# zhizdev/mvdfusion

Hardware: AMD Instinct MI355X
Metric: denoising-steps/sec (higher is better)
Workload: dtype f16x3 (f16 MFMA operands split hi+lo, 3 partial products, fp32 accumulate); 1 GPU; BASELINE.json configs[1]: V=4 views x 256^2 images (32x32 latents), D=1, 50-step DDIM (eta 1), cfg 2.5, SD1.x UNet 320ch + 10 view-aligned transformers + GridAttn, random-init (deterministic fill) weights; views=4, latent=32, depth_samples=1, parallelism=single GPU, CFG pair batched as 2V, hipgraph=True, gemm_tuning=mvdfusion_amd/tuned/gemm_f16.json: 426 problems; 0 problems tuned in this run

## Files before the change

### include/mvd_hip.h

```cpp
#ifndef MVD_HIP_H
#define MVD_HIP_H
#include <stddef.h>
#include <stdint.h>
#ifdef __cplusplus
extern "C" {
#endif

typedef void* mvd_stream_t;

#define MVD_VERSION 100
#define MVD_PREC_X1 1
#define MVD_PREC_X3 3
#define MVD_PREC_X4 4

int mvd_version(void);
const char* mvd_last_error(void);
int mvd_operand_format(void);

size_t mvd_packed_weight_bytes(int N, int K);
int mvd_pack_linear_weight(const float* w, int N, int K, int ldw, int geglu, float scale, void* packed,
                           mvd_stream_t stream);
int mvd_pack_linear_weight_t(const float* wt, int N, int K, int ldw, float scale, void* packed, mvd_stream_t stream);
int mvd_pack_conv3x3_weight(const float* w, int Cout, int Cin, int cin_pad, float scale, void* packed,
                            mvd_stream_t stream);
// ... 119 lines not shown

int mvd_pixel_cross_attn(const float* q, const float* k, const float* v, void* out_sp, int P, int D, int heads,
                         int dhead, mvd_stream_t stream);

int mvd_unet_input(const float* x, const float* input_latents, void* out_sp, int V, int S, int cpad, int cfg,
                   mvd_stream_t stream);
int mvd_unet_input_scenes(const float* x, const float* input_latents, void* out_sp, int nscene, int V, int S, int cpad, int cfg,
                          mvd_stream_t stream);
int mvd_concat_channels(const float* a, int Ca, const float* b, int Cb, float* out, void* out_sp, int rows, long long* gn_stats,
                        int gn_hw, int gn_groups, mvd_stream_t stream);
int mvd_concat_groupnorm_fits(int Ca, int Cb, int hw, int groups);
int mvd_concat_groupnorm(const float* a, int Ca, const float* b, int Cb, float* out, void* raw_sp, void* y_sp, const float* gamma,
                         const float* beta, long long* gn_stats, int B, int hw, int groups, float eps, int silu, mvd_stream_t stream);
int mvd_area_pool(const float* vol, void* out_sp, int B, int S, int D, int C, int factor, int ldp, mvd_stream_t stream);
int mvd_fill_zero(float* p, size_t n, mvd_stream_t stream);

#define MVD_STEP_STRIDE 8
int mvd_timestep_embedding(const float* steps, const int* iter, const float* freqs, float* out, int dim,
                           mvd_stream_t stream);
int mvd_timestep_embedding_scenes(const float* steps, const int* iter, const float* freqs, float* out, int dim, int nscene,
                                  int steps_scene_stride, mvd_stream_t stream);
int mvd_advance_iter(int* iter, mvd_stream_t stream);

#define MVD_CAM_RECORD 20
#define MVD_TOKEN_DIM 723
#define MVD_TOKEN_LD 736
int mvd_zembed(const float* lat, const float* w, const float* b, float* feat, int N, int S, mvd_stream_t stream);
int mvd_gridattn_tokens(const float* x, const float* depth_noise, const float* steps, const int* iter,
                        const float* grid_lin ,
                        const float* feat, const float* in_feat, const float* cams, const float* in_cam,
                        void* tokens_sp, int V, int q0, int Vq, int S, int D, float depth_scale, float depth_shift,
                        mvd_stream_t stream);
int mvd_gridattn_tokens_scenes(const float* x, const float* depth_noise, const float* steps, const int* iter, const float* grid_lin,
                               const float* feat, const float* in_feat, const float* cams, const float* in_cam, void* tokens_sp,
                               int nscene, int V, int q0, int Vq, int S, int D, float depth_scale, float depth_shift,
                               mvd_stream_t stream);
int mvd_gridattn_tokens_scenes_t(const float* x, const float* depth_noise, const float* steps, const int* iter, const float* grid_lin,
                                 const float* feat, const float* in_feat, const float* cams, const float* in_cam, void* tokens_sp,
                                 int nscene, int V, int q0, int Vq, int S, int D, float depth_scale, float depth_shift,
                                 int steps_scene_stride, mvd_stream_t stream);
int mvd_gridattn_fused_slots(void);
size_t mvd_gridattn_fused_stream_bytes(void);
size_t mvd_gridattn_fused_vec_floats(void);
int mvd_gridattn_fused(const float* x, const float* depth_noise, const float* steps, const int* iter, const float* grid_lin,
                       const float* feat, const float* in_feat, const float* cams, const float* in_cam, const void* wstream,
                       const float* vecs, void* pooled_sp, int V, int q0, int Vq, int S, int D, float depth_scale,
// ... 305 lines not shown
```

### mvdfusion_amd/csrc/elementwise.hip

```cpp
#include "common.hpp"
#include "../../include/mvd_hip.h"

namespace {

__device__ __forceinline__ float act_apply(float v, int act) {
  if (act == MVD_ACT_GELU) return gelu_erf(v);
  if (act == MVD_ACT_SILU) return silu_f(v);
  return v;
}

template <int MR>
__global__ __launch_bounds__(256) void gemv_kernel(const float* __restrict__ W, const float* __restrict__ bias,
                                                   const float* __restrict__ x, float* __restrict__ y, int M, int N, int K, int ldx,
                                                   int ldy, int act_in, int act_out) {
  const int lane = threadIdx.x & 63;
  const int n = blockIdx.x * 4 + (threadIdx.x >> 6);
  if (n >= N) return;
  float acc[MR];
#pragma unroll
  for (int m = 0; m < MR; ++m) acc[m] = 0.f;
  const float* wr = W + (size_t)n * K;
  if ((K & 3) == 0) {
    for (int k = lane * 4; k < K; k += 256) {
      const float4 w4 = *(const float4*)(wr + k);
// ... 266 lines not shown
        acc.z += v.z;
        acc.w += v.w;
      }
    store_sp4(out_sp, e / C4, ldp, c * 4, acc.x * inv, acc.y * inv, acc.z * inv, acc.w * inv);
  }
}

__global__ __launch_bounds__(256) void fill_zero_kernel(float* p, size_t n) {
  for (size_t e = (size_t)blockIdx.x * 256 + threadIdx.x; e < n; e += (size_t)gridDim.x * 256) p[e] = 0.f;
}

__global__ void timestep_embedding_kernel(const float* __restrict__ steps, const int* __restrict__ iter,
                                          const float* __restrict__ freqs, float* __restrict__ out, int dim, int steps_scene_stride) {
  const float t = steps[((size_t)iter[0] + (size_t)blockIdx.x * steps_scene_stride) * MVD_STEP_STRIDE + 0];
  out += (size_t)blockIdx.x * dim;
  const int half = dim / 2;
  for (int i = threadIdx.x; i < half; i += blockDim.x) {
    const float a = t * freqs[i];
    out[i] = cosf(a);
    out[half + i] = sinf(a);
  }
}

__global__ void advance_iter_kernel(int* iter) {
  if (threadIdx.x == 0) iter[0] += 1;
}

__global__ __launch_bounds__(256) void cfg_ddim_kernel(const float* __restrict__ eps_nhwc, int ldc, float* __restrict__ x,
                                                       float* __restrict__ x0, float* __restrict__ eps_out,
                                                       const float* __restrict__ noise, const float* __restrict__ steps,
                                                       const int* __restrict__ iter, int V, int S, int cfg, float cfg_scale,
                                                       int do_update, size_t noise_stride) {
  const int it = iter[0];
  const float* st = steps + (size_t)it * MVD_STEP_STRIDE;
  const float a_t = st[3], a_prev = st[4], sigma = st[5], s1m = st[6], has_noise = st[7];
  const int SS = S * S;
  const size_t total = (size_t)V * 5 * SS;
  for (size_t e = (size_t)blockIdx.x * 256 + threadIdx.x; e < total; e += (size_t)gridDim.x * 256) {
    const int pix = (int)(e % SS);
    const int c = (int)((e / SS) % 5);
    const int b = (int)(e / ((size_t)5 * SS));
    float ep = eps_nhwc[((size_t)b * SS + pix) * ldc + c];
    if (cfg) {
      const float eu = eps_nhwc[((size_t)(V + b) * SS + pix) * ldc + c];
      ep = eu + cfg_scale * (ep - eu);
    }
// ... 54 lines not shown
  if (b > (size_t)cap) b = cap;
  if (b < 1) b = 1;
  return (int)b;
}

}

extern "C" int mvd_gemv(const float* W, const float* bias, const float* x, float* y, int M, int N, int K, int ldx, int ldy,
                        int act_in, int act_out, mvd_stream_t stream) {
  MVD_CHECK_ARG(W && x && y && M > 0 && M <= 16 && N > 0 && K > 0, "mvd_gemv: bad arguments (M <= 16)");
  if ((K & 3) == 0) MVD_CHECK_ARG((ldx & 3) == 0, "mvd_gemv: ldx must be a multiple of 4 when K is");
  hipStream_t s = (hipStream_t)stream;
  dim3 grid(cdiv(N, 4)), block(256);
  if (M <= 1)
    hipLaunchKernelGGL(gemv_kernel<1>, grid, block, 0, s, W, bias, x, y, M, N, K, ldx, ldy, act_in, act_out);
  else if (M <= 4)
    hipLaunchKernelGGL(gemv_kernel<4>, grid, block, 0, s, W, bias, x, y, M, N, K, ldx, ldy, act_in, act_out);
  else
    hipLaunchKernelGGL(gemv_kernel<16>, grid, block, 0, s, W, bias, x, y, M, N, K, ldx, ldy, act_in, act_out);
  MVD_CHECK_LAUNCH("mvd_gemv");
  return 0;
}

extern "C" int mvd_unet_input_scenes(const float* x, const float* input_latents, void* out_sp, int nscene, int V, int S, int cpad, int cfg,
                                     mvd_stream_t stream) {
  MVD_CHECK_ARG(x && input_latents && out_sp && cpad % 32 == 0 && V > 0 && S > 0 && cpad >= 10, "mvd_unet_input: bad arguments");
  MVD_CHECK_ARG(nscene >= 1 && (long long)nscene * V <= 0x3fffffff, "mvd_unet_input_scenes: nscene=%d (>= 1)", nscene);
  const int NV = nscene * V;
  const int nb = cfg ? 2 * NV : NV;
  const size_t total = (size_t)nb * S * S * cpad;
  hipLaunchKernelGGL(unet_input_kernel, dim3(grid_for(total)), dim3(256), 0, (hipStream_t)stream, x, input_latents, (u16*)out_sp, NV, V,
                     S, cpad, nb);
  MVD_CHECK_LAUNCH("mvd_unet_input");
  return 0;
}

extern "C" int mvd_unet_input(const float* x, const float* input_latents, void* out_sp, int V, int S, int cpad, int cfg,
                              mvd_stream_t stream) {
  return mvd_unet_input_scenes(x, input_latents, out_sp, 1, V, S, cpad, cfg, stream);
}

extern "C" int mvd_concat_channels(const float* a, int Ca, const float* b, int Cb, float* out, void* out_sp, int rows,
                                   long long* gn_stats, int gn_hw, int gn_groups, mvd_stream_t stream) {
  if (out_sp) MVD_CHECK_ARG((Ca + Cb) % 32 == 0, "mvd_concat_channels: split-planes output needs (Ca+Cb) %% 32 == 0");
  MVD_CHECK_ARG(a && b && out && rows > 0 && Ca > 0 && Cb > 0 && Ca % 4 == 0 && Cb % 4 == 0,
                "mvd_concat_channels: bad arguments (channel counts must be multiples of 4)");
// ... 59 lines not shown
  if (n == 0) return 0;
  hipLaunchKernelGGL(fill_zero_kernel, dim3(grid_for(n)), dim3(256), 0, (hipStream_t)stream, p, n);
  MVD_CHECK_LAUNCH("mvd_fill_zero");
  return 0;
}

extern "C" int mvd_timestep_embedding(const float* steps, const int* iter, const float* freqs, float* out, int dim,
                                      mvd_stream_t stream) {
  MVD_CHECK_ARG(steps && iter && freqs && out && dim > 0 && dim % 2 == 0, "mvd_timestep_embedding: bad arguments");
  hipLaunchKernelGGL(timestep_embedding_kernel, dim3(1), dim3(256), 0, (hipStream_t)stream, steps, iter, freqs, out, dim, 0);
  MVD_CHECK_LAUNCH("mvd_timestep_embedding");
  return 0;
}

extern "C" int mvd_timestep_embedding_scenes(const float* steps, const int* iter, const float* freqs, float* out, int dim, int nscene,
                                             int steps_scene_stride, mvd_stream_t stream) {
  MVD_CHECK_ARG(steps && iter && freqs && out && dim > 0 && dim % 2 == 0, "mvd_timestep_embedding: bad arguments");
  MVD_CHECK_ARG(nscene >= 1 && nscene <= 65535 && steps_scene_stride >= 0 && (nscene > 1 || steps_scene_stride == 0),
                "mvd_timestep_embedding_scenes: nscene=%d (1 ... 65535), steps_scene_stride=%d (>= 0; 0 when nscene = 1)", nscene,
                steps_scene_stride);
  hipLaunchKernelGGL(timestep_embedding_kernel, dim3(nscene), dim3(256), 0, (hipStream_t)stream, steps, iter, freqs, out, dim,
                     steps_scene_stride);
  MVD_CHECK_LAUNCH("mvd_timestep_embedding_scenes");
  return 0;
}

extern "C" int mvd_advance_iter(int* iter, mvd_stream_t stream) {
  MVD_CHECK_ARG(iter != nullptr, "mvd_advance_iter: null pointer");
  hipLaunchKernelGGL(advance_iter_kernel, dim3(1), dim3(64), 0, (hipStream_t)stream, iter);
  MVD_CHECK_LAUNCH("mvd_advance_iter");
  return 0;
}

extern "C" int mvd_cfg_ddim_update(const float* eps_nhwc, int ldc, float* x, float* x0, float* eps_out,
                                   const float* ddim_noise, size_t noise_stride, const float* steps, const int* iter, int V,
                                   int S, int cfg, float cfg_scale, int do_update, mvd_stream_t stream) {
  MVD_CHECK_ARG(eps_nhwc && steps && iter && V > 0 && S > 0 && ldc >= 5, "mvd_cfg_ddim_update: bad arguments");
  if (do_update) MVD_CHECK_ARG(x && x0 && ddim_noise, "mvd_cfg_ddim_update: update needs x, x0, ddim_noise");
  const size_t total = (size_t)V * 5 * S * S;
  hipLaunchKernelGGL(cfg_ddim_kernel, dim3(grid_for(total)), dim3(256), 0, (hipStream_t)stream, eps_nhwc, ldc, x, x0, eps_out,
                     ddim_noise, steps, iter, V, S, cfg, cfg_scale, do_update, noise_stride);
  MVD_CHECK_LAUNCH("mvd_cfg_ddim_update");
  return 0;
}

extern "C" int mvd_pin_views(float* x, float* x0, const float* known, const float* noise, size_t noise_stride, const float* steps,
// ... 26 lines not shown
```

### mvdfusion_amd/hip.py

```python
import ctypes as C
import os

import torch

_HERE = os.path.dirname(os.path.abspath(__file__))
LIB_PATHS = {"f16": os.path.join(_HERE, "csrc", "libmvd_hip.so"), "bf16": os.path.join(_HERE, "csrc", "libmvd_hip_bf16.so")}
if os.environ.get("MVD_HIP_LIB"):
    LIB_PATHS["f16"] = os.environ["MVD_HIP_LIB"]
LIB_PATH = LIB_PATHS["f16"]
OPERAND_FORMAT = os.environ.get("MVD_OPERAND_FORMAT", "f16")

PREC_X1, PREC_X3, PREC_X4 = 1, 3, 4
PREC_KINDS = ("conv", "skip", "proj", "qkv", "attn", "out", "geglu", "ffproj", "xattn", "ga")


def parse_precision(name):
    base, _, over = name.partition(":")
    names = {"f16": ("f16", PREC_X1), "bf16": ("bf16", PREC_X1), "f16x3": ("f16", PREC_X3), "f16x4": ("f16", PREC_X4),
             "bf16x3": ("bf16", PREC_X3), "bf16x4": ("bf16", PREC_X4)}
    if base not in names:
        raise ValueError(f"precision '{name}': base must be one of {sorted(names)}")
    fmt, default = names[base]
    policy = {}
    for item in filter(None, over.split(",")):
# ... 118 lines not shown
    "mvd_gridattn_tokens_backward": (_i, [_vp, _vp, _vp, _vp, _vp, _vp, _vp, _vp, _i, _vp, _vp, _f, _i, _i, _i, _i, _i, _f, _f, _vp]),
    "mvd_gridattn_tokens_backward_scenes": (_i, [_vp, _vp, _vp, _vp, _vp, _vp, _vp, _vp, _i, _vp, _vp, _f, _i, _i, _i, _i, _i, _i, _f, _f, _i,
                                                 _vp]),
    "mvd_gridattn_tokens_backward_window": (_i, [_vp, _vp, _vp, _vp, _vp, _vp, _vp, _vp, _i, _vp, _vp, _f, _i, _i, _i, _i, _i, _i, _f, _f, _i,
                                                 _i, _vp]),
    "mvd_layernorm_backward": (_i, [_vp, _vp, _vp, _i, _i, _f, _vp, _vp, _vp]),
    "mvd_layernorm_backward_groups": (_i, [_vp, _vp, _vp, _i, _i, _i, _i, _f, _vp, _vp, _vp, _vp, _vp, _sz, _vp]),
    "mvd_geglu_backward": (_i, [_vp, _vp, _i, _i, _vp, _vp]),
    "mvd_act_planes": (_i, [_vp, _vp, _vp, _sz, _i, _i, _i, _i, _i, _vp]),
    "mvd_act_backward": (_i, [_vp, _vp, _vp, _sz, _i, _vp]),
    "mvd_attention_backward": (_i, [_vp, _vp, _vp, _vp, _i, _i, _i, _i, _vp, _vp, _vp, _vp, _sz, _vp]),
    "mvd_pixel_cross_attn_backward": (_i, [_vp, _vp, _vp, _vp, _i, _i, _i, _i, _vp, _vp, _vp, _vp]),
    "mvd_groupnorm_backward": (_i, [_vp, _vp, _vp, _vp, _i, _i, _i, _i, _f, _i, _vp, _vp, _vp, _vp, _sz, _vp]),
    "mvd_groupnorm_from_stats": (_i, [_vp, _vp, _vp, _vp, _vp, _i, _i, _i, _i, _f, _i, _vp]),
    "mvd_area_pool": (_i, [_vp, _vp, _i, _i, _i, _i, _i, _i, _vp]),
    "mvd_fill_zero": (_i, [_vp, _sz, _vp]),
    "mvd_pow2_scale": (_i, [_vp, _sz, _vp, _vp, _vp]),
    "mvd_split_planes_scaled": (_i, [_vp, _vp, _sz, _i, _i, _i, _vp, _vp]),
    "mvd_transpose_planes_scaled": (_i, [_vp, _i, _i, _i, _vp, _i, _vp, _vp]),
    "mvd_adamw_multi": (_i, [_vp, _i, _i, _f, _f, _f, _f, _f, _f, _f, _f, _vp]),
    "mvd_timestep_embedding": (_i, [_vp, _vp, _vp, _vp, _i, _vp]),
    "mvd_timestep_embedding_scenes": (_i, [_vp, _vp, _vp, _vp, _i, _i, _i, _vp]),
    "mvd_advance_iter": (_i, [_vp, _vp]),
    "mvd_zembed": (_i, [_vp, _vp, _vp, _vp, _i, _i, _vp]),
    "mvd_gridattn_tokens": (_i, [_vp] * 10 + [_i, _i, _i, _i, _i, _f, _f, _vp]),
    "mvd_gridattn_tokens_scenes": (_i, [_vp] * 10 + [_i, _i, _i, _i, _i, _i, _f, _f, _vp]),
    "mvd_gridattn_tokens_scenes_t": (_i, [_vp] * 10 + [_i, _i, _i, _i, _i, _i, _f, _f, _i, _vp]),
    "mvd_gridattn_fused_slots": (_i, []),
    "mvd_gridattn_fused_stream_bytes": (_sz, []),
    "mvd_gridattn_fused_vec_floats": (_sz, []),
    "mvd_gridattn_fused": (_i, [_vp] * 12 + [_i, _i, _i, _i, _i, _f, _f, _i, _vp]),
    "mvd_gridattn_fused_scenes": (_i, [_vp] * 12 + [_i, _i, _i, _i, _i, _i, _f, _f, _i, _vp]),
    "mvd_gridattn_fused_scenes_t": (_i, [_vp] * 12 + [_i, _i, _i, _i, _i, _i, _f, _f, _i, _i, _i, _vp]),
    "mvd_gridattn_tokens_window": (_i, [_vp] * 10 + [_i, _i, _i, _i, _i, _i, _f, _f, _i, _i, _vp]),
    "mvd_gridattn_fused_window": (_i, [_vp] * 12 + [_i, _i, _i, _i, _i, _i, _f, _f, _i, _i, _i, _i, _vp]),
    "mvd_view_mha": (_i, [_vp, _vp, _i, _i, _i, _i, _vp]),
    "mvd_view_pool": (_i, [_vp, _vp, _vp, _vp, _i, _i, _i, _vp]),
    "mvd_cfg_ddim_update": (_i, [_vp, _i, _vp, _vp, _vp, _vp, _sz, _vp, _vp, _i, _i, _i, _f, _i, _vp]),
    "mvd_pin_views": (_i, [_vp, _vp, _vp, _vp, _sz, _vp, _vp, _i, _i, _i, _i, _i, _vp]),
    "mvd_fuse_points": (_i, [_vp] * 9 + [_i, _i, _i, _i, _f, _f, _f, _f, _f, _i, _vp]),
    "mvd_compact_points_scratch": (_sz, [_sz]),
    "mvd_compact_points": (_i, [_vp] * 5 + [_sz, _i, _i, _vp, _vp, _vp, _vp, _vp, _vp, _sz, _vp]),
    "mvd_render_points_scratch": (_sz, [_i, _i]),
    "mvd_render_points": (_i, [_vp] * 4 + [_sz, _i, _i, _i, _i, _f, _f, C.POINTER(_f), _vp, _vp, _vp, _vp, _sz, _vp]),
    "mvd_render_points_stages": (_i, [_vp] * 4 + [_sz, _i, _i, _i, _i, _f, _f, C.POINTER(_f), _vp, _vp, _vp, _vp, _sz, _i, _vp]),
    "mvd_render_mesh_scratch": (_sz, [_i, _i]),
# ... 897 lines not shown
```

### mvdfusion_amd/unet.py

```python
import math

import torch
import torch.nn as nn

from . import hip
from .attention import SpatialTransformer, ViewAlignedFeatureTransformer
from .engine import Ctx


class GroupNorm32(nn.GroupNorm):
    pass


def normalization(channels):
    return GroupNorm32(32, channels)


class TimestepBlock(nn.Module):
    pass


class Upsample(nn.Module):
    def __init__(self, channels, use_conv, dims=2, out_channels=None, padding=1):
        super().__init__()
# ... 196 lines not shown
        self._head = None
        self._temb = None
        self._xattn = None
        self._head_saved = None
        self._record = None

    def get_cross_attn_parameters(self, finetune_cross_attn, finetune_view_attn):
        out = []
        for name, p in self.named_parameters():
            if finetune_cross_attn and any(k in name for k in (".norm.", ".proj_in.", ".transformer_blocks.", ".proj_out.")):
                out.append(p)
            if finetune_view_attn and ".aligned_attn_" in name:
                out.append(p)
        return out

    def disable_unet_grad(self):
        for name, p in self.named_parameters():
            if ".aligned_attn_" not in name:
                p.requires_grad_(False)

    def _resblocks(self):
        return [m for m in self.modules() if isinstance(m, ResBlock)]

    def time_biases(self, ctx, t_sin):
        if self._temb is None:
            blocks = self._resblocks()
            w = torch.cat([b.emb_layers[1].weight.detach() for b in blocks], 0).contiguous()
            bias = torch.cat([b.emb_layers[1].bias.detach() + b.in_layers[2].bias.detach() for b in blocks], 0).contiguous()
            offs, o = {}, 0
            for b in blocks:
                offs[b] = (o, o + b.out_channels)
                o += b.out_channels
            self._temb = (w, bias, offs)
        w, bias, offs = self._temb
        ted = self.model_channels * 4
        R = t_sin.shape[0]
        e1, emb = ctx.ws.get("temb.e1", (R, ted)), ctx.ws.get("temb.emb", (R, ted))
        out = ctx.ws.get("temb.bias", (R, w.shape[0]))
        ctx.gemv_rows(self.time_embed[0].weight, self.time_embed[0].bias, t_sin, e1, act_out=hip.ACT_SILU)
        ctx.gemv_rows(self.time_embed[2].weight, self.time_embed[2].bias, e1, emb)
        ctx.gemv_rows(w, bias, emb, out, act_in=hip.ACT_SILU)
        ctx.emb_bias = {b: out[:, lo:hi] for b, (lo, hi) in offs.items()}

    def cross_attn_vectors(self, ctx):
        if self._xattn is None:
            sts = [m for m in self.modules() if isinstance(m, SpatialTransformer)]
            ws, bs, offs, o = [], [], {}, 0
            for st in sts:
                a2 = st.transformer_blocks[0].attn2
                wo, wv = a2.to_out[0].weight.detach().double(), a2.to_v.weight.detach().double()
                ws.append((wo @ wv).float())
                bs.append(a2.to_out[0].bias.detach().float())
                offs[st] = (o, o + st.in_channels)
                o += st.in_channels
            self._xattn = (torch.cat(ws, 0).contiguous(), torch.cat(bs, 0).contiguous(), offs, o)
        w, bias, offs, total = self._xattn
        out = ctx.ws.get("xattn.vec", (ctx.context.shape[0], total))
        ctx.gemv_rows(w, bias, ctx.context, out)
        ctx.xattn_vec = {st: out[:, lo:hi] for st, (lo, hi) in offs.items()}

    def run(self, ctx, x_in, t_sin, S):
        B = ctx.B
        self.time_biases(ctx, t_sin)
        self.cross_attn_vectors(ctx)
        hs = []
        H = W = S
        h = x_in
        rec = self._record
        for bi, blk in enumerate(self.input_blocks):
            if rec is not None:
                rec.append((blk, h.clone(), H, W, 0))
            if bi == 0:
                o = ctx.ws.get("hs0", (B * H * W, self.model_channels))
                ctx.next_gn = gn_hint(self.input_blocks[1][0])
                h = blk[0].run(ctx, h, H, W, o)
                ctx.next_gn = None
            else:
                last = blk[-1]
                Ho, Wo = (H // 2, W // 2) if isinstance(last, Downsample) else (H, W)
                co = last.out_channels if isinstance(last, (ResBlock, Downsample)) else last.in_channels
                o = ctx.ws.get(f"hs{bi}", (B * Ho * Wo, co))
                nxt = self.input_blocks[bi + 1][0] if bi + 1 < len(self.input_blocks) else self.middle_block[0]
                h, H, W = blk.run(ctx, h, H, W, out=o, next_layer=nxt)
            hs.append((h, H, W))
        if rec is not None:
            rec.append((self.middle_block, h.clone(), H, W, 0))
        keep = rec is not None or ctx.keep_fp32
# ... 94 lines not shown
```

### mvdfusion_amd/viewfusion_zero_depth_rgb.py

```python
import math

import torch
import torch.nn as nn

from . import hip
from .cameras import Cameras, get_camera_slice, get_relative_camera, pack_cameras
from .engine import Ctx, ddim_step_table
from .sampler import DDIMSampler
from .scheduler import DDPMScheduler
from .unet import UNetWrapper
from .view_attn_efficient2 import GridAttn

import os

PREFETCH_WEIGHTS = os.environ.get("MVD_PREFETCH", "ws")
PREFETCH_OPTIONS = {k: int(v) for k, v in (kv.split("=") for kv in os.environ.get("MVD_PREFETCH_OPTS", "").split(",") if kv)}


def _sinusoid_freqs(dim, max_period=10000):
    half = dim // 2
    return torch.exp(-math.log(max_period) * torch.arange(start=0, end=half, dtype=torch.float32) / half)


class StepEngine:
# ... 15 lines not shown
        self.eps = z(NV, 5, S, S)
        self.input_latents = z(N, 5, S, S)
        self.clip_v_embed = z(NV, 796)
        self.cams = z(NV, hip.CAM_RECORD)
        self.in_cam = z(N, hip.CAM_RECORD)
        self.context = z(B, 768)
        self.vol = z(B * S * S * D, 768)
        self.vol_planes, self.vol_col = model.unet_model.level0_operand(self.ctx, B, S, D)
        self.x_in = torch.zeros(B * S * S, 2 * 32, dtype=torch.int16, device=dev)
        self.iter = torch.zeros(1, dtype=torch.int32, device=dev)
        self.steps = z(1, hip.STEP_STRIDE)
        self.steps_nodiv = z(1, hip.STEP_STRIDE)
        self.prev = z(NV, 5, S, S)
        self.depth_mode = 0
        self.pin = None
        self.known = z(1, 5, S, S)
        self.pin_noise = None
        self.depth_noise = z(1, NV, D, S, S)
        self.ddim_noise = z(1, NV, 5, S, S)
        self.f256 = _sinusoid_freqs(256).to(dev)
        self.funet = _sinusoid_freqs(model.unet_model.unet_model.model_channels).to(dev)
        self.graphs = {}
        self.prefetchers = {}
        self.drop_masks = None
        self.n_rows = 1
        self.steps_scene_stride = 0
        self.done = 0

    def set_conditioning(self, batch_cameras, input_latents, input_cameras, clip_v_embed):
        self.set_conditioning_scenes([(batch_cameras, input_latents, input_cameras, clip_v_embed)])

    def set_conditioning_scenes(self, conds):
        if len(conds) != self.N:
            raise ValueError(f"set_conditioning_scenes: {len(conds)} scenes for a {self.N}-scene engine")
        V, S = self.V, self.S
        for n, (bc, il, ic, ce) in enumerate(conds):
            self.cams[n * V:(n + 1) * V].copy_(pack_cameras(bc).to(self.cams.device))
            self.in_cam[n:n + 1].copy_(pack_cameras(ic).to(self.cams.device))
            self.input_latents[n:n + 1].copy_(il.reshape(1, 5, S, S))
            self.clip_v_embed[n * V:(n + 1) * V].copy_(ce.reshape(V, 796))

    def set_schedule(self, steps_table, depth_noise, ddim_noise):
        self._set_tables(steps_table, depth_noise, ddim_noise, scene_stride=0)

    def set_schedule_scenes(self, steps_table, depth_noise, ddim_noise=None):
        if self.cfg:
            raise ValueError("StepEngine.set_schedule_scenes: per-scene timesteps need a cfg=False engine (the training step); "
                             "guided sampling steps share one timestep")
        if tuple(steps_table.shape) != (self.N, hip.STEP_STRIDE):
            raise ValueError(f"StepEngine.set_schedule_scenes: step table {tuple(steps_table.shape)} for {self.N} scenes "
                             f"(expected ({self.N}, {hip.STEP_STRIDE}))")
        if ddim_noise is None:
            ddim_noise = torch.zeros(1, self.N * self.V, 5, self.S, self.S)
        self._set_tables(steps_table, depth_noise, ddim_noise, scene_stride=1 if self.N > 1 else 0)

    def _set_tables(self, steps_table, depth_noise, ddim_noise, scene_stride):
        dev = self.ctx.device
        if self.steps.shape != steps_table.shape:
            self.graphs.clear()
            self.prefetchers.clear()
            self.steps = steps_table.to(dev).contiguous()
            self.steps_nodiv = self.steps.clone()
            self.depth_noise = depth_noise.to(dev).contiguous()
            self.ddim_noise = ddim_noise.to(dev).contiguous()
        else:
            self.steps.copy_(steps_table)
            self.depth_noise.copy_(depth_noise)
            self.ddim_noise.copy_(ddim_noise)
        self.steps_nodiv.copy_(self.steps)
        self.steps_nodiv[:, 1] = 1.0
        self.steps_scene_stride = scene_stride
        self.n_rows = int(steps_table.shape[0]) - (self.N - 1) * scene_stride
        self.rewind()

    def set_pin(self, mode, known, noise=None):
        dev = self.ctx.device
        nk = int(known.shape[0])
        K = nk // self.N
        if mode not in (0, 1) or K < 1 or K * self.N != nk or K > self.V or tuple(known.shape[1:]) != (5, self.S, self.S):
            raise ValueError(f"StepEngine.set_pin: mode {mode}, known {tuple(known.shape)} for {self.N} scene(s) of {self.V} views at "
                             f"S = {self.S} (expected (N*K, 5, S, S), 1 <= K <= V)")
        if mode == 1 and (noise is None or tuple(noise.shape) != (int(self.steps.shape[0]), nk, 5, self.S, self.S)):
            raise ValueError(f"StepEngine.set_pin: mode 1 needs noise ({int(self.steps.shape[0])}, {nk}, 5, {self.S}, {self.S}), got "
                             f"{None if noise is None else tuple(noise.shape)}")
        if self.known.shape != known.shape:
            self.graphs.clear()
            self.prefetchers.clear()
            self.known = known.to(dev, torch.float32).contiguous().clone()
        else:
            self.known.copy_(known)
        if mode == 1:
            if self.pin_noise is None or self.pin_noise.shape != noise.shape:
                self.graphs.clear()
                self.prefetchers.clear()
# ... 10 lines not shown
        self.iter.fill_(it)
        self.done = it

    def depth_geo(self):
        if self.depth_mode == 0:
            return self.x, self.steps
        return (self.x0 if self.depth_mode == 1 else self.prev), self.steps_nodiv

    def enqueue(self, cfg_scale, do_update, prefetcher=None):
        m, ctx, L = self.m, self.ctx, hip.lib()
        V, S, D, B, q0, Vq, N = self.V, self.S, self.D, self.B, self.q0, self.Vq, self.N
        NVq = N * Vq
        ctx.B, ctx.D = B, D
        ctx.begin_step()
        st = hip.stream
        sst, R = self.steps_scene_stride, self.t_rows
        if sst and do_update:
            raise ValueError("StepEngine: per-scene timesteps (set_schedule_scenes) are a training step: no DDIM update")
        if self.pin is not None:
            mode, K = self.pin
            pn = self.pin_noise if mode == 1 else None
            hip.check(L.mvd_pin_views(hip.ptr(self.x), hip.ptr(self.x0), hip.ptr(self.known), hip.ptr(pn), N * K * 5 * S * S,
                                      hip.ptr(self.steps), hip.ptr(self.iter), N, V, K, S, mode, st()))
        ts = ctx.ws.get("vf.tsin", (R, 256))
        te1 = ctx.ws.get("vf.te1", (R, 256))
        c = ctx.ws.get("vf.c", (R, 256))
        hip.check(L.mvd_timestep_embedding_scenes(hip.ptr(self.steps), hip.ptr(self.iter), hip.ptr(self.f256), hip.ptr(ts), 256, R, sst,
                                                  st()))
        ctx.gemv_rows(m.time_embed[0].weight, m.time_embed[0].bias, ts, te1, act_out=hip.ACT_SILU)
        ctx.gemv_rows(m.time_embed[2].weight, m.time_embed[2].bias, te1, c)
        dsrc, dsteps = self.depth_geo()
        m.view_attn.run(ctx, self.x, self.depth_noise, self.steps, self.iter, self.cams, self.in_cam,
                        self.input_latents, c, self.vol, V, S, D, q0=q0, Vq=Vq, vol_planes=self.vol_planes,
                        vol_planes_col=self.vol_col, depth_src=None if self.depth_mode == 0 else dsrc,
                        depth_steps=None if self.depth_mode == 0 else dsteps, scenes=N, steps_scene_stride=sst)
        p = m.cc_projection
        c1 = ctx.ws.get("vf.cc1", (NVq, 768))
        c2 = ctx.ws.get("vf.cc2", (NVq, 768))
        ctx.gemv_rows(p[0].weight, p[0].bias, self.clip_v_embed[q0:q0 + NVq], c1, act_out=hip.ACT_SILU)
        ctx.gemv_rows(p[2].weight, p[2].bias, c1, c2, act_out=hip.ACT_SILU)
        ctx.gemv_rows(p[4].weight, p[4].bias, c2, self.context[:NVq])
        if self.drop_masks is not None:
            clip_m, vol_m, cat_m = self.drop_masks
            self.context[:NVq] *= clip_m[:, None]
            self.vol.view(B, -1)[:NVq] *= vol_m[:, None]
            vp = self.vol_planes.view(B, S * S * D, -1)
            vp[:NVq, :, 2 * self.vol_col:] *= vol_m.to(torch.int16)[:, None, None]
        ctx.context = self.context
        xq, x0q, epsq = self.x[q0:q0 + NVq], self.x0[q0:q0 + NVq], self.eps[q0:q0 + NVq]
        hip.check(L.mvd_unet_input_scenes(hip.ptr(xq), hip.ptr(self.input_latents), hip.ptr(self.x_in), N, Vq, S, 32,
                                          int(self.cfg), st()))
        if self.drop_masks is not None:
            xin = self.x_in.view(B, S * S, 64)
            cm = self.drop_masks[2].to(torch.int16)[:, None, None]
            xin[:NVq, :, 5:10] *= cm
            xin[:NVq, :, 37:42] *= cm
        unet = m.unet_model.unet_model
        ctx.vol_levels = m.unet_model.volume_pyramid(ctx, self.vol.view(B, S, S, D, 768), B, S, D)
        tsu = ctx.ws.get("vf.tsin_unet", (R, unet.model_channels))
        hip.check(L.mvd_timestep_embedding_scenes(hip.ptr(self.steps), hip.ptr(self.iter), hip.ptr(self.funet), hip.ptr(tsu),
                                                  unet.model_channels, R, sst, st()))
        y = unet.run(ctx, self.x_in, tsu, S)
        hip.check(L.mvd_cfg_ddim_update(hip.ptr(y), 8, hip.ptr(xq), hip.ptr(x0q), hip.ptr(epsq),
                                        hip.ptr(self.ddim_noise[:, q0:q0 + NVq]), N * V * 5 * S * S, hip.ptr(self.steps),
                                        hip.ptr(self.iter), NVq, S, int(self.cfg), float(cfg_scale), int(do_update), st()))
        if do_update:
            hip.check(L.mvd_advance_iter(hip.ptr(self.iter), st()))

    @property
    def t_rows(self):
        return self.N if self.steps_scene_stride else 1

    def step(self, cfg_scale, do_update, use_graph=True):
        key = (float(cfg_scale), bool(do_update), int(self.depth_mode), self.steps_scene_stride, self.pin)
        if self.done >= self.n_rows:
            raise IndexError(f"StepEngine.step: iteration {self.done} is past the {self.n_rows}-row step table "
                             "(set_schedule() / rewind() before stepping again)")
        if do_update:
            self.done += 1
        if not use_graph:
            return self.enqueue(cfg_scale, do_update)
        g = self.graphs.get(key)
        if g is None:
            it0 = self.iter.clone()
            x_keep, x0_keep = self.x.clone(), self.x0.clone()
            hip.AUTOTUNE = True
            try:
                self.enqueue(cfg_scale, do_update)
            finally:
                hip.AUTOTUNE = False
                hip.release_tuning_buffers()
            torch.cuda.synchronize()
            pf = None
            if PREFETCH_WEIGHTS == "ws":
                pf = hip.WeightPrefetcher(self.x.device, **PREFETCH_OPTIONS)
                self.iter.copy_(it0)
                self.x.copy_(x_keep)
                self.x0.copy_(x0_keep)
                with pf.following(record=True):
                    self.enqueue(cfg_scale, do_update)
                torch.cuda.synchronize()
            self.iter.copy_(it0)
            self.x.copy_(x_keep)
            self.x0.copy_(x0_keep)
# ... 100 lines not shown
                prm.requires_grad_(False)
        self.cc_projection = nn.Sequential(nn.Linear(768 + 14 * 2, 768), nn.SiLU(True), nn.Linear(768, 768),
                                           nn.SiLU(True), nn.Linear(768, 768))
        nn.init.eye_(list(self.cc_projection.parameters())[0][:768, :768])
        nn.init.zeros_(list(self.cc_projection.parameters())[1])
        self.time_embed_dim = 256
        self.time_embed = nn.Sequential(nn.Linear(256, 256), nn.SiLU(True), nn.Linear(256, 256))
        self.register_buffer("_device", torch.tensor([0.0]), persistent=False)
        self.latent_size = int(self.view_attn.input_size)
        self.ddim = DDIMSampler(self, ddim_num_steps=50, ddim_discretize="uniform", ddim_eta=1.0,
                                latent_size=self.latent_size, z_dim=4, feed_prev_depth=feed_prev_depth,
                                overwrite_x_noisy=overwrite_x_noisy)
        self._engines = {}
        self._packed_sig = None
        assert self.finetune_view_attn is True, "must finetune new view attention layers"

    train_autotune_min_flops = 2.0e9

    def invalidate_packed(self, keep_engines=False):
        hip.drop_packed_caches(self)
        hip.forget_param_maxima()
        if keep_engines:
            for e in self._engines.values():
                e.graphs.clear()
                e.prefetchers.clear()
        else:
            self._engines.clear()

    def load_state_dict(self, state_dict, strict=True, **kw):
        r = super().load_state_dict(state_dict, strict=strict, **kw)
        self.invalidate_packed()
        self._packed_sig = None
        return r

    def _apply(self, fn, *a, **kw):
        r = super()._apply(fn, *a, **kw)
        if "_engines" in self.__dict__:
            self.invalidate_packed()
            self._packed_sig = None
        return r

    def engine(self, V, S, D, cfg, q0=0, Vq=None, scenes=1):
        if int(scenes) < 1:
            raise ValueError(f"engine(scenes={scenes}): at least one scene")
        if int(scenes) > 1 and (q0 != 0 or (Vq is not None and Vq != V)):
            raise ValueError(f"engine(V={V}, q0={q0}, Vq={Vq}, scenes={scenes}): view-parallel sharding is single-scene only")
        sig = hip.params_signature(self)
        if sig != self._packed_sig:
# ... 425 lines not shown
```

Before: 119.5 steps/s.

## Precompute per-step timestep embedding tables and hoist constant conditioning vectors out of graph

Adds a per-schedule step table that precomputes, for every DDIM row, the outer time-embedding MLP output, the UNet time embedding and all ResBlock time biases. Each captured step then only copies the current iteration's row with one small select kernel instead of running several timestep-embedding and GEMV launches. The CLIP conditioning projection and cross-attention vectors do not change across steps, so they are computed once outside the graph and reused until the weights change. This removes many small launches per step but adds signature tracking and cache invalidation that must be kept correct.

```diff
diff --git a/include/mvd_hip.h b/include/mvd_hip.h
--- a/include/mvd_hip.h
+++ b/include/mvd_hip.h
@@ -165,6 +165,15 @@
                                   int steps_scene_stride, mvd_stream_t stream);
 int mvd_advance_iter(int* iter, mvd_stream_t stream);
 
+int mvd_cond_vectors(const float* clip, int ld_clip, int rows, int k_in, int width, const float* w0, const float* b0, const float* w2,
+                     const float* b2, const float* w4, const float* b4, float* h1, float* h2, float* context, const float* wx,
+                     const float* bx, int nx, int ctx_rows, float* xvec, mvd_stream_t stream);
+int mvd_step_table(const float* steps, const int* row0, int n_rows, const float* freqs, int dim, int hidden, const float* w0,
+                   const float* b0, const float* w2, const float* b2, const float* w3, const float* b3, int n3, float* tsin, float* h,
+                   float* emb, float* out3, mvd_stream_t stream);
+int mvd_select_step_rows(const int* iter, int n_rows, const float* t0, float* d0, int w0, const float* t1, float* d1, int w1,
+                         const float* t2, float* d2, int w2, mvd_stream_t stream);
+
 #define MVD_CAM_RECORD 20
 #define MVD_TOKEN_DIM 723
 #define MVD_TOKEN_LD 736
diff --git a/mvdfusion_amd/csrc/elementwise.hip b/mvdfusion_amd/csrc/elementwise.hip
--- a/mvdfusion_amd/csrc/elementwise.hip
+++ b/mvdfusion_amd/csrc/elementwise.hip
@@ -312,6 +312,26 @@
   }
 }
 
+__global__ __launch_bounds__(256) void select_step_rows_kernel(const int* __restrict__ iter, int n_rows, const float4* __restrict__ t0,
+                                                               float4* __restrict__ d0, int w0, const float4* __restrict__ t1,
+                                                               float4* __restrict__ d1, int w1, const float4* __restrict__ t2,
+                                                               float4* __restrict__ d2, int w2) {
+  const int r = iter[0];
+  if (r < 0 || r >= n_rows) return;
+  int e = blockIdx.x * 256 + threadIdx.x;
+  if (e < w0) {
+    d0[e] = t0[(size_t)r * w0 + e];
+    return;
+  }
+  e -= w0;
+  if (e < w1) {
+    d1[e] = t1[(size_t)r * w1 + e];
+    return;
+  }
+  e -= w1;
+  if (e < w2) d2[e] = t2[(size_t)r * w2 + e];
+}
+
 __global__ void advance_iter_kernel(int* iter) {
   if (threadIdx.x == 0) iter[0] += 1;
 }
@@ -412,6 +432,30 @@
   return 0;
 }
 
+static int gemv_rows(const float* W, const float* bias, const float* x, float* y, int rows, int N, int K, int ldx, int ldy, int act_in,
+                     int act_out, mvd_stream_t stream) {
+  for (int r = 0; r < rows; r += 16) {
+    const int rc = mvd_gemv(W, bias, x + (size_t)r * ldx, y + (size_t)r * ldy, rows - r < 16 ? rows - r : 16, N, K, ldx, ldy, act_in,
+                            act_out, stream);
+    if (rc) return rc;
+  }
+  return 0;
+}
+
+extern "C" int mvd_cond_vectors(const float* clip, int ld_clip, int rows, int k_in, int width, const float* w0, const float* b0,
+                                const float* w2, const float* b2, const float* w4, const float* b4, float* h1, float* h2, float* context,
+                                const float* wx, const float* bx, int nx, int ctx_rows, float* xvec, mvd_stream_t stream) {
+  MVD_CHECK_ARG(clip && w0 && w2 && w4 && h1 && h2 && context && wx && xvec, "mvd_cond_vectors: null pointer");
+  MVD_CHECK_ARG(rows > 0 && k_in > 0 && width > 0 && nx > 0 && ctx_rows >= rows && ld_clip >= k_in,
+                "mvd_cond_vectors: rows=%d k_in=%d width=%d nx=%d ctx_rows=%d (>= rows) ld_clip=%d (>= k_in)", rows, k_in, width, nx,
+                ctx_rows, ld_clip);
+  int rc = gemv_rows(w0, b0, clip, h1, rows, width, k_in, ld_clip, width, MVD_ACT_NONE, MVD_ACT_SILU, stream);
+  if (!rc) rc = gemv_rows(w2, b2, h1, h2, rows, width, width, width, width, MVD_ACT_NONE, MVD_ACT_SILU, stream);
+  if (!rc) rc = gemv_rows(w4, b4, h2, context, rows, width, width, width, width, MVD_ACT_NONE, MVD_ACT_NONE, stream);
+  if (!rc) rc = gemv_rows(wx, bx, context, xvec, ctx_rows, nx, width, width, nx, MVD_ACT_NONE, MVD_ACT_NONE, stream);
+  return rc;
+}
+
 extern "C" int mvd_unet_input_scenes(const float* x, const float* input_latents, void* out_sp, int nscene, int V, int S, int cpad, int cfg,
                                      mvd_stream_t stream) {
   MVD_CHECK_ARG(x && input_latents && out_sp && cpad % 32 == 0 && V > 0 && S > 0 && cpad >= 10, "mvd_unet_input: bad arguments");
@@ -517,6 +561,35 @@
   hipLaunchKernelGGL(timestep_embedding_kernel, dim3(nscene), dim3(256), 0, (hipStream_t)stream, steps, iter, freqs, out, dim,
                      steps_scene_stride);
   MVD_CHECK_LAUNCH("mvd_timestep_embedding_scenes");
+  return 0;
+}
+
+extern "C" int mvd_step_table(const float* steps, const int* row0, int n_rows, const float* freqs, int dim, int hidden, const float* w0,
+                              const float* b0, const float* w2, const float* b2, const float* w3, const float* b3, int n3, float* tsin,
+                              float* h, float* emb, float* out3, mvd_stream_t stream) {
+  MVD_CHECK_ARG(steps && row0 && freqs && w0 && w2 && tsin && h && emb, "mvd_step_table: null pointer");
+  MVD_CHECK_ARG(n_rows >= 1 && n_rows <= 65535 && dim > 0 && dim % 2 == 0 && hidden > 0, "mvd_step_table: n_rows=%d (1 ... 65535) dim=%d hidden=%d",
+                n_rows, dim, hidden);
+  MVD_CHECK_ARG((w3 == nullptr) == (out3 == nullptr) && (w3 == nullptr || n3 > 0), "mvd_step_table: w3 / out3 / n3 go together");
+  int rc = mvd_timestep_embedding_scenes(steps, row0, freqs, tsin, dim, n_rows, n_rows > 1 ? 1 : 0, stream);
+  if (!rc) rc = gemv_rows(w0, b0, tsin, h, n_rows, hidden, dim, dim, hidden, MVD_ACT_NONE, MVD_ACT_SILU, stream);
+  if (!rc) rc = gemv_rows(w2, b2, h, emb, n_rows, hidden, hidden, hidden, hidden, MVD_ACT_NONE, MVD_ACT_NONE, stream);
+  if (!rc && w3) rc = gemv_rows(w3, b3, emb, out3, n_rows, n3, hidden, hidden, n3, MVD_ACT_SILU, MVD_ACT_NONE, stream);
+  return rc;
+}
+
+extern "C" int mvd_select_step_rows(const int* iter, int n_rows, const float* t0, float* d0, int w0, const float* t1, float* d1, int w1,
+                                    const float* t2, float* d2, int w2, mvd_stream_t stream) {
+  MVD_CHECK_ARG(iter && n_rows >= 1 && t0 && d0 && w0 > 0 && w1 >= 0 && w2 >= 0, "mvd_select_step_rows: bad arguments");
+  MVD_CHECK_ARG((w1 == 0 || (t1 && d1)) && (w2 == 0 || (t2 && d2)), "mvd_select_step_rows: a table with a width needs both pointers");
+  MVD_CHECK_ARG((w0 & 3) == 0 && (w1 & 3) == 0 && (w2 & 3) == 0 && (long long)w0 + w1 + w2 <= 0x3fffffff,
+                "mvd_select_step_rows: widths %d %d %d must be multiples of 4", w0, w1, w2);
+  MVD_CHECK_ARG((((uintptr_t)t0 | (uintptr_t)d0 | (uintptr_t)t1 | (uintptr_t)d1 | (uintptr_t)t2 | (uintptr_t)d2) & 15) == 0,
+                "mvd_select_step_rows: 16-byte alignment");
+  const int total = (w0 + w1 + w2) / 4;
+  hipLaunchKernelGGL(select_step_rows_kernel, dim3(cdiv(total, 256)), dim3(256), 0, (hipStream_t)stream, iter, n_rows, (const float4*)t0,
+                     (float4*)d0, w0 / 4, (const float4*)t1, (float4*)d1, w1 / 4, (const float4*)t2, (float4*)d2, w2 / 4);
+  MVD_CHECK_LAUNCH("mvd_select_step_rows");
   return 0;
 }
 
diff --git a/mvdfusion_amd/hip.py b/mvdfusion_amd/hip.py
--- a/mvdfusion_amd/hip.py
+++ b/mvdfusion_amd/hip.py
@@ -164,6 +164,9 @@
     "mvd_timestep_embedding": (_i, [_vp, _vp, _vp, _vp, _i, _vp]),
     "mvd_timestep_embedding_scenes": (_i, [_vp, _vp, _vp, _vp, _i, _i, _i, _vp]),
     "mvd_advance_iter": (_i, [_vp, _vp]),
+    "mvd_cond_vectors": (_i, [_vp, _i, _i, _i, _i, _vp, _vp, _vp, _vp, _vp, _vp, _vp, _vp, _vp, _vp, _vp, _i, _i, _vp, _vp]),
+    "mvd_step_table": (_i, [_vp, _vp, _i, _vp, _i, _i, _vp, _vp, _vp, _vp, _vp, _vp, _i, _vp, _vp, _vp, _vp, _vp]),
+    "mvd_select_step_rows": (_i, [_vp, _i, _vp, _vp, _i, _vp, _vp, _i, _vp, _vp, _i, _vp]),
     "mvd_zembed": (_i, [_vp, _vp, _vp, _vp, _i, _i, _vp]),
     "mvd_gridattn_tokens": (_i, [_vp] * 10 + [_i, _i, _i, _i, _i, _f, _f, _vp]),
     "mvd_gridattn_tokens_scenes": (_i, [_vp] * 10 + [_i, _i, _i, _i, _i, _i, _f, _f, _vp]),
diff --git a/mvdfusion_amd/unet.py b/mvdfusion_amd/unet.py
--- a/mvdfusion_amd/unet.py
+++ b/mvdfusion_amd/unet.py
@@ -242,7 +242,7 @@
     def _resblocks(self):
         return [m for m in self.modules() if isinstance(m, ResBlock)]
 
-    def time_biases(self, ctx, t_sin):
+    def temb_weights(self):
         if self._temb is None:
             blocks = self._resblocks()
             w = torch.cat([b.emb_layers[1].weight.detach() for b in blocks], 0).contiguous()
@@ -252,17 +252,25 @@
                 offs[b] = (o, o + b.out_channels)
                 o += b.out_channels
             self._temb = (w, bias, offs)
-        w, bias, offs = self._temb
-        ted = self.model_channels * 4
+        return self._temb
+
+    def time_bias_buffers(self, ctx, R):
+        w, _, offs = self.temb_weights()
+        emb = ctx.ws.get("temb.emb", (R, self.model_channels * 4))
+        out = ctx.ws.get("temb.bias", (R, w.shape[0]))
+        ctx.emb_bias = {b: out[:, lo:hi] for b, (lo, hi) in offs.items()}
+        return emb, out
+
+    def time_biases(self, ctx, t_sin):
+        w, bias, _ = self.temb_weights()
         R = t_sin.shape[0]
-        e1, emb = ctx.ws.get("temb.e1", (R, ted)), ctx.ws.get("temb.emb", (R, ted))
-        out = ctx.ws.get("temb.bias", (R, w.shape[0]))
+        e1 = ctx.ws.get("temb.e1", (R, self.model_channels * 4))
+        emb, out = self.time_bias_buffers(ctx, R)
         ctx.gemv_rows(self.time_embed[0].weight, self.time_embed[0].bias, t_sin, e1, act_out=hip.ACT_SILU)
         ctx.gemv_rows(self.time_embed[2].weight, self.time_embed[2].bias, e1, emb)
         ctx.gemv_rows(w, bias, emb, out, act_in=hip.ACT_SILU)
-        ctx.emb_bias = {b: out[:, lo:hi] for b, (lo, hi) in offs.items()}
-
-    def cross_attn_vectors(self, ctx):
+
+    def xattn_weights(self):
         if self._xattn is None:
             sts = [m for m in self.modules() if isinstance(m, SpatialTransformer)]
             ws, bs, offs, o = [], [], {}, 0
@@ -274,15 +282,26 @@
                 offs[st] = (o, o + st.in_channels)
                 o += st.in_channels
             self._xattn = (torch.cat(ws, 0).contiguous(), torch.cat(bs, 0).contiguous(), offs, o)
-        w, bias, offs, total = self._xattn
+        return self._xattn
+
+    def xattn_buffer(self, ctx):
+        _, _, offs, total = self.xattn_weights()
         out = ctx.ws.get("xattn.vec", (ctx.context.shape[0], total))
-        ctx.gemv_rows(w, bias, ctx.context, out)
         ctx.xattn_vec = {st: out[:, lo:hi] for st, (lo, hi) in offs.items()}
+        return out
+
+    def cross_attn_vectors(self, ctx):
+        w, bias, _, _ = self.xattn_weights()
+        ctx.gemv_rows(w, bias, ctx.context, self.xattn_buffer(ctx))
 
     def run(self, ctx, x_in, t_sin, S):
         B = ctx.B
-        self.time_biases(ctx, t_sin)
-        self.cross_attn_vectors(ctx)
+        if t_sin is None:
+            self.time_bias_buffers(ctx, 1)
+            self.xattn_buffer(ctx)
+        else:
+            self.time_biases(ctx, t_sin)
+            self.cross_attn_vectors(ctx)
         hs = []
         H = W = S
         h = x_in
diff --git a/mvdfusion_amd/viewfusion_zero_depth_rgb.py b/mvdfusion_amd/viewfusion_zero_depth_rgb.py
--- a/mvdfusion_amd/viewfusion_zero_depth_rgb.py
+++ b/mvdfusion_amd/viewfusion_zero_depth_rgb.py
@@ -61,7 +61,12 @@
         self.funet = _sinusoid_freqs(model.unet_model.unet_model.model_channels).to(dev)
         self.graphs = {}
         self.prefetchers = {}
-        self.drop_masks = None
+        self.step_tables = os.environ.get("MVD_STEP_TABLES", "1") != "0"
+        self.iter0 = torch.zeros(1, dtype=torch.int32, device=dev)
+        self._tables = None
+        self._cond_sig = None
+        self._tab_sig = None
+        self._drop_masks = None
         self.n_rows = 1
         self.steps_scene_stride = 0
         self.done = 0
@@ -78,6 +83,71 @@
             self.in_cam[n:n + 1].copy_(pack_cameras(ic).to(self.cams.device))
             self.input_latents[n:n + 1].copy_(il.reshape(1, 5, S, S))
             self.clip_v_embed[n * V:(n + 1) * V].copy_(ce.reshape(V, 796))
+        self._cond_sig = None
+
+    @property
+    def drop_masks(self):
+        return self._drop_masks
+
+    @drop_masks.setter
+    def drop_masks(self, masks):
+        self._drop_masks = masks
+        if masks is not None:
+            self._cond_sig = None
+
+    def invalidate(self):
+        self.graphs.clear()
+        self.prefetchers.clear()
+        self._cond_sig = self._tab_sig = None
+
+    def tables_apply(self):
+        return self.step_tables and self.steps_scene_stride == 0 and self._drop_masks is None and not self.ctx.keep_fp32 and \
+            int(self.steps.shape[0]) > 1
+
+    def _model_sig(self):
+        return (getattr(self.m, "_packed_sig", None),)
+
+    def vector_plan(self):
+        if self.tables_apply():
+            return 1, int(self.steps.shape[0])
+        chunks = lambda rows: -(-rows // 16)
+        return 2 + 5 * chunks(self.t_rows) + 3 * chunks(self.N * self.Vq) + chunks(self.B), None
+
+    def vectors_valid(self):
+        sig = self._model_sig()
+        return self.tables_apply() and self._cond_sig == sig and self._tab_sig == sig
+
+    def refresh_vectors(self):
+        m, ctx, L, st = self.m, self.ctx, hip.lib(), hip.stream
+        unet = m.unet_model.unet_model
+        sig = self._model_sig()
+        if self._cond_sig != sig:
+            NVq, p = self.N * self.Vq, m.cc_projection
+            ctx.context = self.context
+            wx, bx, _, nx = unet.xattn_weights()
+            c1, c2 = ctx.ws.get("vf.cc1", (NVq, 768)), ctx.ws.get("vf.cc2", (NVq, 768))
+            clip = self.clip_v_embed[self.q0:self.q0 + NVq]
+            hip.check(L.mvd_cond_vectors(hip.ptr(clip), clip.stride(0), NVq, 796, 768, hip.ptr(p[0].weight), hip.ptr(p[0].bias),
+                                         hip.ptr(p[2].weight), hip.ptr(p[2].bias), hip.ptr(p[4].weight), hip.ptr(p[4].bias), hip.ptr(c1),
+                                         hip.ptr(c2), hip.ptr(self.context), hip.ptr(wx), hip.ptr(bx), nx, self.B,
+                                         hip.ptr(unet.xattn_buffer(ctx)), st()))
+            self._cond_sig = sig
+        if self._tab_sig != sig:
+            n, mc = int(self.steps.shape[0]), unet.model_channels
+            we, be, _ = unet.temb_weights()
+            ted, nb = 4 * mc, int(we.shape[0])
+            T = self._tables
+            if T is None:
+                e = lambda w: torch.empty(n, w, dtype=torch.float32, device=ctx.device)
+                T = self._tables = dict(c=e(256), emb=e(ted), bias=e(nb), tsin=e(256), h=e(256), tsu=e(mc), e1=e(ted))
+            t, u = m.time_embed, unet.time_embed
+            hip.check(L.mvd_step_table(hip.ptr(self.steps), hip.ptr(self.iter0), n, hip.ptr(self.f256), 256, 256, hip.ptr(t[0].weight),
+                                       hip.ptr(t[0].bias), hip.ptr(t[2].weight), hip.ptr(t[2].bias), None, None, 0, hip.ptr(T["tsin"]),
+                                       hip.ptr(T["h"]), hip.ptr(T["c"]), None, st()))
+            hip.check(L.mvd_step_table(hip.ptr(self.steps), hip.ptr(self.iter0), n, hip.ptr(self.funet), mc, ted, hip.ptr(u[0].weight),
+                                       hip.ptr(u[0].bias), hip.ptr(u[2].weight), hip.ptr(u[2].bias), hip.ptr(we), hip.ptr(be), nb,
+                                       hip.ptr(T["tsu"]), hip.ptr(T["e1"]), hip.ptr(T["emb"]), hip.ptr(T["bias"]), st()))
+            self._tab_sig = sig
 
     def set_schedule(self, steps_table, depth_noise, ddim_noise):
         self._set_tables(steps_table, depth_noise, ddim_noise, scene_stride=0)
@@ -102,6 +172,7 @@
             self.steps_nodiv = self.steps.clone()
             self.depth_noise = depth_noise.to(dev).contiguous()
             self.ddim_noise = ddim_noise.to(dev).contiguous()
+            self._tables = None
         else:
             self.steps.copy_(steps_table)
             self.depth_noise.copy_(depth_noise)
@@ -109,6 +180,7 @@
         self.steps_nodiv.copy_(self.steps)
         self.steps_nodiv[:, 1] = 1.0
         self.steps_scene_stride = scene_stride
+        self._tab_sig = None
         self.n_rows = int(steps_table.shape[0]) - (self.N - 1) * scene_stride
         self.rewind()
 
@@ -165,24 +237,33 @@
             pn = self.pin_noise if mode == 1 else None
             hip.check(L.mvd_pin_views(hip.ptr(self.x), hip.ptr(self.x0), hip.ptr(self.known), hip.ptr(pn), N * K * 5 * S * S,
                                       hip.ptr(self.steps), hip.ptr(self.iter), N, V, K, S, mode, st()))
-        ts = ctx.ws.get("vf.tsin", (R, 256))
-        te1 = ctx.ws.get("vf.te1", (R, 256))
+        unet = m.unet_model.unet_model
+        tabs = self.vectors_valid()
         c = ctx.ws.get("vf.c", (R, 256))
-        hip.check(L.mvd_timestep_embedding_scenes(hip.ptr(self.steps), hip.ptr(self.iter), hip.ptr(self.f256), hip.ptr(ts), 256, R, sst,
-                                                  st()))
-        ctx.gemv_rows(m.time_embed[0].weight, m.time_embed[0].bias, ts, te1, act_out=hip.ACT_SILU)
-        ctx.gemv_rows(m.time_embed[2].weight, m.time_embed[2].bias, te1, c)
+        if tabs:
+            T = self._tables
+            emb, bias = unet.time_bias_buffers(ctx, 1)
+            hip.check(L.mvd_select_step_rows(hip.ptr(self.iter), int(T["c"].shape[0]), hip.ptr(T["c"]), hip.ptr(c), 256, hip.ptr(T["emb"]),
+                                             hip.ptr(emb), emb.shape[1], hip.ptr(T["bias"]), hip.ptr(bias), bias.shape[1], st()))
+        else:
+            ts = ctx.ws.get("vf.tsin", (R, 256))
+            te1 = ctx.ws.get("vf.te1", (R, 256))
+            hip.check(L.mvd_timestep_embedding_scenes(hip.ptr(self.steps), hip.ptr(self.iter), hip.ptr(self.f256), hip.ptr(ts), 256, R, sst,
+                                                      st()))
+            ctx.gemv_rows(m.time_embed[0].weight, m.time_embed[0].bias, ts, te1, act_out=hip.ACT_SILU)
+            ctx.gemv_rows(m.time_embed[2].weight, m.time_embed[2].bias, te1, c)
         dsrc, dsteps = self.depth_geo()
         m.view_attn.run(ctx, self.x, self.depth_noise, self.steps, self.iter, self.cams, self.in_cam,
                         self.input_latents, c, self.vol, V, S, D, q0=q0, Vq=Vq, vol_planes=self.vol_planes,
                         vol_planes_col=self.vol_col, depth_src=None if self.depth_mode == 0 else dsrc,
                         depth_steps=None if self.depth_mode == 0 else dsteps, scenes=N, steps_scene_stride=sst)
-        p = m.cc_projection
-        c1 = ctx.ws.get("vf.cc1", (NVq, 768))
-        c2 = ctx.ws.get("vf.cc2", (NVq, 768))
-        ctx.gemv_rows(p[0].weight, p[0].bias, self.clip_v_embed[q0:q0 + NVq], c1, act_out=hip.ACT_SILU)
-        ctx.gemv_rows(p[2].weight, p[2].bias, c1, c2, act_out=hip.ACT_SILU)
-        ctx.gemv_rows(p[4].weight, p[4].bias, c2, self.context[:NVq])
+        if not tabs:
+            p = m.cc_projection
+            c1 = ctx.ws.get("vf.cc1", (NVq, 768))
+            c2 = ctx.ws.get("vf.cc2", (NVq, 768))
+            ctx.gemv_rows(p[0].weight, p[0].bias, self.clip_v_embed[q0:q0 + NVq], c1, act_out=hip.ACT_SILU)
+            ctx.gemv_rows(p[2].weight, p[2].bias, c1, c2, act_out=hip.ACT_SILU)
+            ctx.gemv_rows(p[4].weight, p[4].bias, c2, self.context[:NVq])
         if self.drop_masks is not None:
             clip_m, vol_m, cat_m = self.drop_masks
             self.context[:NVq] *= clip_m[:, None]
@@ -198,11 +279,12 @@
             cm = self.drop_masks[2].to(torch.int16)[:, None, None]
             xin[:NVq, :, 5:10] *= cm
             xin[:NVq, :, 37:42] *= cm
-        unet = m.unet_model.unet_model
         ctx.vol_levels = m.unet_model.volume_pyramid(ctx, self.vol.view(B, S, S, D, 768), B, S, D)
-        tsu = ctx.ws.get("vf.tsin_unet", (R, unet.model_channels))
-        hip.check(L.mvd_timestep_embedding_scenes(hip.ptr(self.steps), hip.ptr(self.iter), hip.ptr(self.funet), hip.ptr(tsu),
-                                                  unet.model_channels, R, sst, st()))
+        tsu = None
+        if not tabs:
+            tsu = ctx.ws.get("vf.tsin_unet", (R, unet.model_channels))
+            hip.check(L.mvd_timestep_embedding_scenes(hip.ptr(self.steps), hip.ptr(self.iter), hip.ptr(self.funet), hip.ptr(tsu),
+                                                      unet.model_channels, R, sst, st()))
         y = unet.run(ctx, self.x_in, tsu, S)
         hip.check(L.mvd_cfg_ddim_update(hip.ptr(y), 8, hip.ptr(xq), hip.ptr(x0q), hip.ptr(epsq),
                                         hip.ptr(self.ddim_noise[:, q0:q0 + NVq]), N * V * 5 * S * S, hip.ptr(self.steps),
@@ -215,7 +297,8 @@
         return self.N if self.steps_scene_stride else 1
 
     def step(self, cfg_scale, do_update, use_graph=True):
-        key = (float(cfg_scale), bool(do_update), int(self.depth_mode), self.steps_scene_stride, self.pin)
+        tabs = self.tables_apply()
+        key = (float(cfg_scale), bool(do_update), int(self.depth_mode), self.steps_scene_stride, self.pin, tabs)
         if self.done >= self.n_rows:
             raise IndexError(f"StepEngine.step: iteration {self.done} is past the {self.n_rows}-row step table "
                              "(set_schedule() / rewind() before stepping again)")
@@ -223,6 +306,8 @@
             self.done += 1
         if not use_graph:
             return self.enqueue(cfg_scale, do_update)
+        if tabs:
+            self.refresh_vectors()
         g = self.graphs.get(key)
         if g is None:
             it0 = self.iter.clone()
@@ -369,8 +454,7 @@
         hip.forget_param_maxima()
         if keep_engines:
             for e in self._engines.values():
-                e.graphs.clear()
-                e.prefetchers.clear()
+                e.invalidate()
         else:
             self._engines.clear()
 
```

Result: faster. 120.9 steps/s, median of 6 (+1.2%).
